# patrickltobing/shallow-wavenet

Hardware: AMD Instinct MI355X
Metric: decoded samples/sec (22.05 kHz Laplacian AR decode, whole job) (higher is better)
Workload: dtype f32

## Files before the change

shallow_wavenet_amd/csrc/swn_decode_bl6w.hip:

```cpp
#include <type_traits>
#include "swn_decode_bl6_common.hpp"
#include "swn_decode_internal.hpp"

namespace {

using namespace swn_bl6;

constexpr int NG = 256;
constexpr int S = 128;
constexpr int O1 = 128;

template <int LPC_, bool EXT_>
struct Tw {
    static constexpr int LPC = LPC_;
    static constexpr bool EXT = EXT_;
    using Ext = Tw<LPC_, true>;
    static constexpr int NO = 2 + LPC_;
    static constexpr int WN = cmax(1, LPC_) + 1;
    static constexpr int ring_len(int l) { return pow2ceil((1 << l) + 1); }
    static constexpr int ring_off(int l) { int o = 0; for (int i = 0; i < l; ++i) o += ring_len(i) * H; return o; }
    static constexpr int PF = L * 2 * H;
    static constexpr int NZC = 64, NZB = 4;
    static constexpr int o_ring = 0;
    static constexpr int o_hcat = o_ring + ring_off(L);
    static constexpr int o_gp = o_hcat + L * H;
    static constexpr int o_bx = o_gp + 2 * PF;
    static constexpr int o_bd = o_bx + L * 2 * H;
    static constexpr int o_old = o_bd + L * 2 * H;
    static constexpr int o_wup = o_old + 2 * L * 2 * H;
    static constexpr int o_skip = o_wup + 256;
    static constexpr int o_p2 = o_skip + S;
    static constexpr int o_tnz = o_p2 + 4 * NO;
    static constexpr int o_cz = o_tnz + r4(NZB * NZC);
    static constexpr int o_w2 = o_cz + 5 * H;
    static constexpr int o_bias = o_w2 + NO * S + r4(NO);
    static constexpr int o_w1 = o_bias + S + O1;
    static constexpr int o_wl = o_w1 + 8 * O1 * 16;
    static constexpr int o_h0w = o_wl + 8 * NG * 4;
    static constexpr int o_end = o_h0w + 3 * H;
    static constexpr size_t lds_bytes = (size_t)o_end * sizeof(float);
    static constexpr int sess_old = ring_off(L);
    static constexpr int sess_win = sess_old + 2 * L * 2 * H;
    static constexpr int sess_floats = sess_win + r4(WN);
};

__device__ __forceinline__ float sum_quads(float v) {
    v += dpp_f<0x124>(v);
    v += dpp_f<0x128>(v);
    float w = v;
    asm("s_nop 1\n\tv_permlane16_swap_b32 %0, %1" : "+v"(v), "+v"(w));
    v += w;
    w = v;
    asm("s_nop 1\n\tv_permlane32_swap_b32 %0, %1" : "+v"(v), "+v"(w));
    return v + w;
}
template <class T, int LAYER>
__device__ __forceinline__ void layer_a(float* lds, const float (&w)[2][16], const int q, const float wj, const int pb, const int po,
                                        const int ta, const float* xr) {
    const int o = ta >> 2, p = ta & 3, pr = p & 1;
    const float e_old = lds[T::o_old + po + LAYER * 2 * H + pr * H + o];
    const float e_gx = fmaf(wj, lds[T::o_gp + pb + LAYER * 2 * H + pr * H + o], lds[T::o_bx + LAYER * 2 * H + pr * H + o]);
    const float e_hp = xr[o];
    float az = 0.f, ac = 0.f;
#pragma unroll
    for (int m = 0; m < 4; ++m) {
        const float4 x = *reinterpret_cast<const float4*>(xr + 16 * p + 4 * m);
        az = fmaf(w[0][4 * m], x.x, az); ac = fmaf(w[1][4 * m], x.x, ac);
        az = fmaf(w[0][4 * m + 1], x.y, az); ac = fmaf(w[1][4 * m + 1], x.y, ac);
        az = fmaf(w[0][4 * m + 2], x.z, az); ac = fmaf(w[1][4 * m + 2], x.z, ac);
        az = fmaf(w[0][4 * m + 3], x.w, az); ac = fmaf(w[1][4 * m + 3], x.w, ac);
    }
    az = sum4(az); ac = sum4(ac);
    __builtin_amdgcn_sched_barrier(0);
    if (p < 2) {
        const float sa = (p == 0 ? az : ac) + e_old;
        const float v = e_gx * sa;
        float res;
        if (fabsf(v) > 9.02f && p == 1) {
            res = copysignf(1.f, v);
        } else {
            const float e = exp_c(p == 0 ? -v : -2.f * fabsf(v));
            const float r = rcp_c(1.f + e);
            res = p == 0 ? r : copysignf((1.f - e) * r, v);
        }
        const float c = dpp_f<0xF5>(res);
        if (p == 0) {
            const float hn = (1.f - res) * c + res * e_hp;
            if (LAYER + 1 < L) {
                constexpr int R2 = T::ring_len(LAYER + 1 < L ? LAYER + 1 : LAYER);
                lds[T::o_ring + T::ring_off(LAYER + 1 < L ? LAYER + 1 : LAYER) + (q & (R2 - 1)) * H + o] = hn;
            }
            lds[T::o_hcat + LAYER * H + o] = hn;
        }
    }
    __builtin_amdgcn_sched_barrier(0);
}

template <class T, int LAYER, int MB = 4>
__device__ __forceinline__ void older_sum(const float* lds, const float (&w)[2][16], const int qn, const int tb, float& az, float& ac) {
    constexpr int dil = 1 << LAYER;
    constexpr int R = T::ring_len(LAYER);
    const int p = tb & 3;
    const float* ring = lds + T::o_ring + T::ring_off(LAYER);
    az = 0.f; ac = 0.f;
#pragma unroll
    for (int m = 0; m < 4; ++m) {
        const float4 x = *reinterpret_cast<const float4*>(ring + ((qn - dil) & (R - 1)) * H + 16 * p + 4 * m);
        float4 w0, w1;
        if (LAYER < L - 1) {
            w0 = make_float4(w[0][4 * m], w[0][4 * m + 1], w[0][4 * m + 2], w[0][4 * m + 3]);
            w1 = make_float4(w[1][4 * m], w[1][4 * m + 1], w[1][4 * m + 2], w[1][4 * m + 3]);
        } else {
            w0 = *reinterpret_cast<const float4*>(lds + T::o_wl + (m * NG + tb) * 4);
            w1 = *reinterpret_cast<const float4*>(lds + T::o_wl + ((4 + m) * NG + tb) * 4);
        }
        az = fmaf(w0.x, x.x, az); ac = fmaf(w1.x, x.x, ac);
        az = fmaf(w0.y, x.y, az); ac = fmaf(w1.y, x.y, ac);
        az = fmaf(w0.z, x.z, az); ac = fmaf(w1.z, x.z, ac);
        az = fmaf(w0.w, x.w, az); ac = fmaf(w1.w, x.w, ac);
        if (MB < 4 && m % MB == MB - 1) __builtin_amdgcn_sched_barrier(0);
    }
    az = sum4(az); ac = sum4(ac);
}
template <class T, int LAYER>
__device__ __forceinline__ void older_store(float* lds, const int qn, const int tb, const float az, const float ac) {
    const int o = tb >> 2, p = tb & 3, pr = p & 1;
    lds[T::o_old + (qn & 1) * (L * 2 * H) + LAYER * 2 * H + pr * H + o] = (p == 0 ? az : ac) + lds[T::o_bd + LAYER * 2 * H + pr * H + o];
}
template <class T, int LAYER, int MB = 4>
__device__ __forceinline__ void older_b(float* lds, const float (&w)[2][16], const int qn, const int tb) {
    float az, ac;
    older_sum<T, LAYER, MB>(lds, w, qn, tb, az, ac);
    if ((tb & 3) < 2) older_store<T, LAYER>(lds, qn, tb, az, ac);
}
template <int... LS> struct Layers {};
template <class T, int NW, int... LS>
__device__ __forceinline__ void older_bn(Layers<LS...>, float* lds, const float (&w)[NW][2][16], const int qn, const int tb) {
    static_assert(((LS < NW) && ...), "register-resident halves only");
    float az[sizeof...(LS)], ac[sizeof...(LS)];
    int k = 0;
    ((older_sum<T, LS>(lds, w[LS], qn, tb, az[k], ac[k]), ++k), ...);
    if ((tb & 3) < 2) {
        k = 0;
        ((older_store<T, LS>(lds, qn, tb, az[k], ac[k]), ++k), ...);
    }
}

template <class T, int LAYER>
__device__ __forceinline__ void older_rows(const float* lds, const int qn, const int tb, float4 (&x)[4]) {
    constexpr int dil = 1 << LAYER;
    constexpr int R = T::ring_len(LAYER);
    const float* row = lds + T::o_ring + T::ring_off(LAYER) + ((qn - dil) & (R - 1)) * H + 16 * (tb & 3);
#pragma unroll
    for (int m = 0; m < 4; ++m) x[m] = *reinterpret_cast<const float4*>(row + 4 * m);
}
__device__ __forceinline__ void older_sum_x(const float (&w)[2][16], const float4 (&x)[4], float& az, float& ac) {
    az = 0.f; ac = 0.f;
#pragma unroll
    for (int m = 0; m < 4; ++m) {
        az = fmaf(w[0][4 * m], x[m].x, az); ac = fmaf(w[1][4 * m], x[m].x, ac);
        az = fmaf(w[0][4 * m + 1], x[m].y, az); ac = fmaf(w[1][4 * m + 1], x[m].y, ac);
        az = fmaf(w[0][4 * m + 2], x[m].z, az); ac = fmaf(w[1][4 * m + 2], x[m].z, ac);
        az = fmaf(w[0][4 * m + 3], x[m].w, az); ac = fmaf(w[1][4 * m + 3], x[m].w, ac);
    }
    az = sum4(az); ac = sum4(ac);
}
template <class T, int... LS>
__device__ __forceinline__ void older_rows_n(Layers<LS...>, const float* lds, const int qn, const int tb, float4 (&x)[sizeof...(LS)][4]) {
    int k = 0;
    ((older_rows<T, LS>(lds, qn, tb, x[k]), ++k), ...);
}
template <class T, int NW, int... LS>
__device__ __forceinline__ void older_bn_x(Layers<LS...>, float* lds, const float (&w)[NW][2][16], const float4 (&x)[sizeof...(LS)][4],
                                           const int qn, const int tb) {
    static_assert(((LS < NW) && ...), "register-resident halves only");
    float az[sizeof...(LS)], ac[sizeof...(LS)];
    int k = 0;
    ((older_sum_x(w[LS], x[k], az[k], ac[k]), ++k), ...);
    if ((tb & 3) < 2) {
        k = 0;
        ((older_store<T, LS>(lds, qn, tb, az[k], ac[k]), ++k), ...);
    }
}

template <int LAYER>
__device__ __forceinline__ void skip_issue_b(__amdgpu_buffer_rsrc_t wsk2, float4 (&wsl)[8], const int tb, const unsigned step0) {
    const int r = tb >> 2, hp = tb & 3;
#pragma unroll
    for (int ps = 0; ps < 2; ++ps)
#pragma unroll
        for (int mm = 0; mm < 4; ++mm)
            wsl[ps * 4 + mm] = buf_ld4(wsk2, (unsigned)((r + 64 * ps) * 4 + hp) * 16u, (unsigned)((LAYER * 4 + mm) * S) * 64u + step0);
}
template <class T, int LAYER>
__device__ __forceinline__ void skip_roll_b(const float* lds, __amdgpu_buffer_rsrc_t wsk2, float4 (&wsl)[8], float (&sacc)[2], const int tb,
                                            const unsigned step0) {
    static_assert(LAYER >= 1 && LAYER < L, "slice LAYER - 1 in flight, slice LAYER to request");
    const int r = tb >> 2, hp = tb & 3;
#pragma unroll
    for (int hf = 0; hf < 2; ++hf) {
#pragma unroll
        for (int mm = 2 * hf; mm < 2 * hf + 2; ++mm) {
            const float4 x = *reinterpret_cast<const float4*>(lds + T::o_hcat + (LAYER - 1) * H + 16 * mm + 4 * hp);
#pragma unroll
            for (int ps = 0; ps < 2; ++ps) {
                const float4 w = wsl[ps * 4 + mm];
                sacc[ps] = fmaf(w.x, x.x, sacc[ps]); sacc[ps] = fmaf(w.y, x.y, sacc[ps]);
                sacc[ps] = fmaf(w.z, x.z, sacc[ps]); sacc[ps] = fmaf(w.w, x.w, sacc[ps]);
            }
        }
        __builtin_amdgcn_sched_barrier(0);
#pragma unroll
        for (int mm = 2 * hf; mm < 2 * hf + 2; ++mm)
#pragma unroll
            for (int ps = 0; ps < 2; ++ps)
                wsl[ps * 4 + mm] = buf_ld4(wsk2, (unsigned)((r + 64 * ps) * 4 + hp) * 16u, (unsigned)((LAYER * 4 + mm) * S) * 64u + step0);
        __builtin_amdgcn_sched_barrier(0);
    }
    asm volatile("" : "+v"(sacc[0]), "+v"(sacc[1]));
}
template <class T>
__device__ __forceinline__ void skip_last_b(float* lds, const float4 (&wsl)[8], const float (&sacc)[2], const int tb) {
    const int r = tb >> 2, hp = tb & 3;
    float part[2][4];
#pragma unroll
    for (int mm = 0; mm < 4; ++mm) {
        const float4 x = *reinterpret_cast<const float4*>(lds + T::o_hcat + (L - 1) * H + 16 * mm + 4 * hp);
#pragma unroll
        for (int ps = 0; ps < 2; ++ps) {
            const float4 w = wsl[ps * 4 + mm];
            part[ps][mm] = fmaf(w.w, x.w, fmaf(w.z, x.z, fmaf(w.y, x.y, w.x * x.x)));
        }
    }
    float s[2];
#pragma unroll
    for (int ps = 0; ps < 2; ++ps) s[ps] = sacc[ps] + ((part[ps][0] + part[ps][1]) + (part[ps][2] + part[ps][3]));
    const float t0 = s[0] + dpp_f<0xB1>(s[0]), t1 = s[1] + dpp_f<0xB1>(s[1]);
    const float v = (hp < 2 ? t0 : t1) + dpp_f<0x4E>(hp < 2 ? t1 : t0);
    if ((hp & 1) == 0) lds[T::o_skip + r + 32 * hp] = fmaxf(v, 0.f);
}

using OlderMerged = Layers<3, 4>;
using OlderOut1 = Layers<0, 1, 2>;

template <class T, bool GA, bool STREAM, bool POOL = false>
__device__ __forceinline__ void decode_body(const Bl6Args& a, float* lds) {
    constexpr bool EXT = T::EXT;
    static_assert(!STREAM || EXT, "streamed chunks run the extended mode");
    constexpr bool grpA = GA;
    const int tid = threadIdx.x, b = POOL ? 0 : blockIdx.x;
    __builtin_assume(GA ? tid < NG : tid >= NG);
    const int tg = tid & (NG - 1);
    const float* __restrict__ P = a.P;
    const int U = a.U;
    const int s0 = STREAM ? a.step0 : 0;
    const bool resume = STREAM && a.resume;
    const int fb0 = STREAM ? s0 / U : 0;

    for (int e = tid; e < T::o_end; e += NT) lds[e] = 0.f;
    __syncthreads();
    for (int e = tid; e < L * 2 * H; e += NT) {
        lds[T::o_bx + e] = P[a.y.bx + e];
        const float bd = P[a.y.bd + e];
        lds[T::o_bd + e] = bd;
        lds[T::o_old + e] = bd;
    }
    for (int e = tid; e < U; e += NT) lds[T::o_wup + e] = P[a.y.wup + e];
    for (int e = tid; e < H; e += NT) lds[T::o_cz + e] = P[a.y.cb + e];
    for (int e = tid; e < S; e += NT) lds[T::o_bias + e] = P[a.y.bsk + e];
    for (int e = tid; e < O1; e += NT) lds[T::o_bias + S + e] = P[a.y.b1 + e];
    for (int e = tid; e < 2 * H; e += NT) { lds[T::o_cz + H + e] = P[a.y.cv + e]; lds[T::o_cz + 3 * H + e] = P[a.y.cc + e]; }
    for (int e = tid; e < T::NO * S; e += NT) lds[T::o_w2 + e] = P[a.y.w2 + (size_t)(e / S) * r4(S) + (e % S)];
    for (int e = tid; e < T::NO; e += NT) lds[T::o_w2 + T::NO * S + e] = P[a.y.b2 + e];
    for (int e = tid; e < 8 * O1 * 16; e += NT) lds[T::o_w1 + e] = P[a.y.w12 + e];
    const __amdgpu_buffer_rsrc_t condr =
        make_rsrc(a.cond + (size_t)b * a.Tf * a.N, (unsigned)((size_t)a.Tf * a.N * sizeof(float)));
    auto load_frame = [&](int fr) {
        float* dst = lds + T::o_gp + (fr & 1) * T::PF;
#pragma unroll
        for (int it = 0; it < (T::PF / 4 + NT - 1) / NT; ++it) {
            const int e4 = it * NT + tid;
            if (e4 < T::PF / 4)
                *reinterpret_cast<float4*>(dst + 4 * e4) =
                    buf_ld4(condr, (unsigned)tid * 16u, (unsigned)(fr * a.N * 4 + it * NT * 16));
        }
    };
    for (int fr = fb0; fr < fb0 + 2 && fr < a.Tf; ++fr) load_frame(fr);
    constexpr int NWR = grpA ? L : L - 1;
    float wreg[NWR][2][16];
    {
        const int o = tg >> 2, p = tg & 3, k = grpA ? 1 : 0;
#pragma unroll
        for (int l = 0; l < L; ++l)
#pragma unroll
            for (int r = 0; r < 2; ++r) {
                const float4* src = reinterpret_cast<const float4*>(P + a.y.wd + (((size_t)l * 2 * H + o + r * H) * 2 + k) * H + 16 * p);
#pragma unroll
                for (int v = 0; v < 4; ++v) {
                    const float4 t = src[v];
                    if (l == L - 1 && !grpA) {
                        *reinterpret_cast<float4*>(lds + T::o_wl + ((r * 4 + v) * NG + tg) * 4) = t;
                    } else {
                        float (&wr)[16] = wreg[l < NWR ? l : 0][r];
                        wr[4 * v] = t.x; wr[4 * v + 1] = t.y; wr[4 * v + 2] = t.z; wr[4 * v + 3] = t.w;
                    }
                }
            }
    }
    __syncthreads();
    const float* sess_b = STREAM ? a.sess + (size_t)b * T::sess_floats : nullptr;
    int tcp = tid;
    asm volatile("" : "+v"(tcp));
    if (resume) {
        for (int e = tcp; e < T::ring_off(L); e += NT) lds[T::o_ring + e] = sess_b[e];
        for (int e = tcp; e < 2 * L * 2 * H; e += NT) lds[T::o_old + e] = sess_b[T::sess_old + e];
        __syncthreads();
    }

    int fb = fb0, tb0 = fb0 * U;
    const int n_pro = RF;
    auto cond_taps = [&](int q, float& wj, int& pb) {
        const int t0 = q - RF;
        const int tlo = t0 < 0 ? 0 : t0;
        if (tlo >= tb0 + U) {
            fb += 1; tb0 += U;
            if (fb + 1 < a.Tf) load_frame(fb + 1);
        }
        int rel = tlo - tb0;
        int fsel = fb;
        if (rel >= U) { rel -= U; fsel = fb + 1; }
        rel = rel < U ? rel : U - 1;
        wj = lds[T::o_wup + rel];
        pb = (fsel & 1) * T::PF;
    };

    auto input_seed = [&](int q) {
        if (tid < H) {
            const int o = tid;
            float acc = c_b;
#pragma unroll
            for (int k = 0; k < 2; ++k) {
                const int r = q - (1 - k);
                if (r >= 0) acc += fmaf(k ? c_v1 : c_v0, 0.f, k ? c_c1 : c_c0);
            }
            lds[T::o_ring + (q & 1) * H + o] = ssign(acc);
        }
    };
    float win[T::WN];
#pragma unroll
    for (int k = 0; k < T::WN; ++k) win[k] = 0.f;
    if (EXT && a.seed) win[T::WN - 1] = reinterpret_cast<const float*>(a.seed)[b];
    if (resume) {
#pragma unroll
        for (int k = 0; k < T::WN; ++k) win[k] = sess_b[T::sess_win + k];
    }
    const int wv = __builtin_amdgcn_readfirstlane(tg >> 6);
    float kcb = 0.f, kv0 = 0.f, kv1 = 0.f, kc0 = 0.f, kc1 = 0.f;
    if (grpA) { const int o = tg & (H - 1); kcb = c_b; kv0 = c_v0; kv1 = c_v1; kc0 = c_c0; kc1 = c_c1; }
    auto h0_row = [&](int qn) -> int {
        return wv == 0 ? T::o_ring + (qn & 1) * H : T::o_h0w + (wv - 1) * H;
    };
    auto input_gen = [&](int row) {
        if constexpr (grpA) {
            float acc = kcb;
            acc += fmaf(kv0, win[T::WN - 2], kc0);
            acc += fmaf(kv1, win[T::WN - 1], kc1);
            lds[row + (tg & (H - 1))] = ssign(acc);
            lds_fence_compiler();
        }
    };
    float e_next = 0.f;
    auto noise_load = [&](int c) {
        const int step = c * T::NZC + tid - 64;
        if (step < a.n_steps) e_next = a.noise[(size_t)b * a.n_steps + step];
    };
    auto noise_chunk = [&](int c) {
        if (grpA && tid >= 64 && tid < 128) {
            const int k = tid - 64, step = c * T::NZC + k;
            if (step < a.n_steps) {
                const float e = EXT ? swn_noise_laplace_at(a.nz, b, step, s0 + step, 0, a.n_steps, 1) : e_next;
                const float sg = (e > 0.f) ? 1.f : ((e < 0.f) ? -1.f : 0.f);
                lds[T::o_tnz + (c & (T::NZB - 1)) * T::NZC + k] = sg * log1pf(-2.f * fabsf(e));
            }
            if (!EXT) noise_load(c + 1);
        }
    };
    if (!EXT && grpA && tid >= 64 && tid < 128) noise_load(0);
    noise_chunk(0);
    noise_chunk(1);

    const __amdgpu_buffer_rsrc_t wsk2 = make_rsrc(P + a.y.wsk2, (unsigned)(L * S * 64 * sizeof(float)));

#ifdef SWN_STAMP
    unsigned long long tw[9] = {0, 0, 0, 0, 0, 0, 0, 0, 0}, tv[6] = {0, 0, 0, 0, 0, 0}, tstep = 0, tlast = 0, tbeg = 0;
#define SWN_BAR(k) { tw[k] += __builtin_amdgcn_s_memtime() - tlast; lds_barrier(); tlast = __builtin_amdgcn_s_memtime(); }
#define SWN_WAIT_STAMP(k) { asm volatile("" :: "v"(wsl[0].x)); tv[k] += __builtin_amdgcn_s_memtime() - tlast; }
#define SWN_PRE(k) { tw[k] += __builtin_amdgcn_s_memtime() - tlast; asm volatile("s_waitcnt lgkmcnt(0)" ::: "memory"); }
#define SWN_BAR_KEEP(k, N) { lds_barrier_keep<N>(); tlast = __builtin_amdgcn_s_memtime(); }
#else
#define SWN_BAR(k) lds_barrier();
#define SWN_WAIT_STAMP(k)
#define SWN_PRE(k)
#define SWN_BAR_KEEP(k, N) lds_barrier_keep<N>();
#endif
#define SWN_PHASE(LAYER, GEN, X0)                                                                                     \
    if constexpr (grpA) layer_a<T, LAYER>(lds, wreg[LAYER], q, wj, pb, po, tg,                                         \
                                          LAYER == 0 ? (X0) : lds + T::o_ring + T::ring_off(LAYER) +                   \
                                                                  (q & (T::ring_len(LAYER) - 1)) * H);                 \
    else {                                                                                                             \
        if (GEN) {    \
                      \
                      \
            if (LAYER == 0) skip_issue_b<0>(wsk2, wsl, tg, step0);                                                     \
            else { SWN_WAIT_STAMP(LAYER > 0 ? LAYER - 1 : 0) skip_roll_b<T, (LAYER > 0 ? LAYER : 1)>(lds, wsk2, wsl, sacc, tg, step0); } \
            __builtin_amdgcn_sched_barrier(0);                                                                         \
        }                                                                                                              \
        if (!(GEN)) older_b<T, LAYER>(lds, wreg[LAYER < NWR ? LAYER : 0], q + 1, tg);                                  \
        else if (LAYER == 0) older_bn<T>(OlderMerged{}, lds, wreg, q + 1, tg);                                         \
        __builtin_amdgcn_sched_barrier(0);                                                                             \
    }                                                                                                                  \
    if (GEN) { SWN_BAR(LAYER) } else lds_barrier();

#pragma unroll 1
    for (int q = resume ? n_pro : 0; q < n_pro; ++q) {
        float wj; int pb;
        float4 wsl[8]; float sacc[2]; const unsigned step0 = 0;
        cond_taps(q, wj, pb);
        const int po = (q & 1) * (L * 2 * H);
        input_seed(q);
        lds_barrier();
        const float* x0 = lds + T::o_ring + (q & 1) * H;
        SWN_PHASE(0, false, x0) SWN_PHASE(1, false, x0) SWN_PHASE(2, false, x0) SWN_PHASE(3, false, x0)
        SWN_PHASE(4, false, x0) SWN_PHASE(5, false, x0)
        (void)wsl; (void)sacc; (void)step0;
    }

    int rel_c = s0 - fb0 * U;
    bool fill_c = false;
    float wj_c = 0.f;
    int pb_c = 0, po_c = 0, x0_c = 0;
    auto taps_ahead = [&](int qn) {
        wj_c = lds[T::o_wup + rel_c];
        pb_c = (fb & 1) * T::PF;
        po_c = (qn & 1) * (L * 2 * H);
        x0_c = h0_row(qn);
        asm volatile("" : "+s"(pb_c), "+s"(po_c), "+s"(x0_c));
    };
    auto frame_advance = [&]() {
        rel_c += 1;
        const bool cross = rel_c >= U;
        if (cross) { rel_c = 0; fb += 1; }
        fill_c = cross && fb + 1 < a.Tf;
    };
    if constexpr (grpA) taps_ahead(RF + s0);
    input_gen(x0_c);
#ifdef SWN_STAMP
    tlast = tbeg = __builtin_amdgcn_s_memtime();
#endif
    auto gen_step = [&](const int i) __attribute__((always_inline)) {
        const int q = RF + s0 + i;
        const float wj = wj_c;
        const int pb = pb_c, po = po_c;
        if constexpr (grpA) {
            if (fill_c) load_frame(fb + 1);
        }
        float4 wsl[8];
        float sacc[2] = {0.f, 0.f};
        if constexpr (!grpA) {
            const float bs0 = lds[T::o_bias + (tg >> 2)], bs1 = lds[T::o_bias + (tg >> 2) + 64];
            if ((tg & 3) == 0) { sacc[0] = bs0; sacc[1] = bs1; }
        }
        unsigned step0 = 0;
        asm volatile("" : "+s"(step0));
        const float* x0 = lds + x0_c;
        SWN_PHASE(0, true, x0) SWN_PHASE(1, true, x0) SWN_PHASE(2, true, x0) SWN_PHASE(3, true, x0)
        SWN_PHASE(4, true, x0) SWN_PHASE(5, true, x0)
        constexpr bool ROLL1 = T::LPC == 0;
        float4 xo[3][4];
        float4 w1e[2][2];
        if constexpr (!grpA) {
            SWN_WAIT_STAMP(5) skip_last_b<T>(lds, wsl, sacc, tg);
            SWN_PRE(6)
            lds_fence_compiler();
            __builtin_amdgcn_sched_barrier(0);
            older_rows_n<T>(OlderOut1{}, lds, q + 1, tg, xo);
            __builtin_amdgcn_sched_barrier(0);
            SWN_BAR_KEEP(6, 12)
        } else {
            older_b<T, L - 1, 2>(lds, wreg[L - 1], q + 1, tg + (int)step0);
            if constexpr (ROLL1) {
                SWN_PRE(6)
                lds_fence_compiler();
                __builtin_amdgcn_sched_barrier(0);
#pragma unroll
                for (int mm = 0; mm < 2; ++mm)
#pragma unroll
                    for (int r = 0; r < 2; ++r)
                        w1e[mm][r] = *reinterpret_cast<const float4*>(lds + T::o_w1 + ((mm * O1 + (tg >> 2) + 64 * r) * 4 + (tg & 3)) * 4);
                __builtin_amdgcn_sched_barrier(0);
                SWN_BAR_KEEP(6, 4)
            } else {
                SWN_BAR(6)
            }
        }
        if constexpr (grpA) {
            const int hr = tg >> 2, hp = tg & 3;
            float a0 = 0.f, a1 = 0.f, b0 = 0.f, b1 = 0.f;
            auto X = [&](int mm) { return *reinterpret_cast<const float4*>(lds + T::o_skip + 16 * mm + 4 * hp); };
            auto W = [&](int mm, int r) { return *reinterpret_cast<const float4*>(lds + T::o_w1 + ((mm * O1 + hr + 64 * r) * 4 + hp) * 4); };
            auto fma8 = [&](int mm, const float4& x0, const float4& w0, const float4& w1) {
                float& acc = (mm & 1) ? a1 : a0;
                float& bcc = (mm & 1) ? b1 : b0;
                acc = fmaf(w0.x, x0.x, acc); acc = fmaf(w0.y, x0.y, acc); acc = fmaf(w0.z, x0.z, acc); acc = fmaf(w0.w, x0.w, acc);
                bcc = fmaf(w1.x, x0.x, bcc); bcc = fmaf(w1.y, x0.y, bcc); bcc = fmaf(w1.z, x0.z, bcc); bcc = fmaf(w1.w, x0.w, bcc);
            };
            float e_b1[2] = {0.f, 0.f}, e_w2[2] = {0.f, 0.f}, e_b2 = 0.f;
            const int e_kc = hp < T::NO ? hp : T::NO - 1;
            if constexpr (ROLL1) {
                static_assert(T::NO <= 4, "one round of out_2 rows");
                float4 xr[3] = {X(0), X(1), X(2)};
                __builtin_amdgcn_sched_barrier(0);
#pragma unroll
                for (int mm = 0; mm < 8; ++mm) {
                    fma8(mm, xr[mm % 3], w1e[mm % 2][0], w1e[mm % 2][1]);
                    __builtin_amdgcn_sched_barrier(0);
                    if (mm + 2 < 8) { w1e[mm % 2][0] = W(mm + 2, 0); w1e[mm % 2][1] = W(mm + 2, 1); }
                    if (mm + 3 < 8) xr[mm % 3] = X(mm + 3);
                    if (mm == 5) {
                        e_b1[0] = lds[T::o_bias + S + hr]; e_b1[1] = lds[T::o_bias + S + hr + 64];
                        e_w2[0] = lds[T::o_w2 + e_kc * S + hr]; e_w2[1] = lds[T::o_w2 + e_kc * S + hr + 64];
                    }
                    if (mm == 6) e_b2 = lds[T::o_w2 + T::NO * S + e_kc];
                    __builtin_amdgcn_sched_barrier(0);
                }
            } else {
#pragma unroll
                for (int mm = 0; mm < 8; ++mm) {
                    fma8(mm, X(mm), W(mm, 0), W(mm, 1));
                    if ((mm & 3) == 3) __builtin_amdgcn_sched_barrier(0);
                }
            }
            const float v = sum4(a0 + a1), u = sum4(b0 + b1);
            if constexpr (ROLL1) {
                const float o1a = fmaxf(v + e_b1[0], 0.f), o1b = fmaxf(u + e_b1[1], 0.f);
                const float pz = sum_quads(fmaf(e_w2[1], o1b, fmaf(e_w2[0], o1a, tg < 4 ? e_b2 : 0.f)));
                if ((tg & 63) < 4 && hp < T::NO) lds[T::o_p2 + 4 * hp + wv] = pz;
            } else {
                const float o1a = fmaxf(v + lds[T::o_bias + S + hr], 0.f), o1b = fmaxf(u + lds[T::o_bias + S + hr + 64], 0.f);
#pragma unroll
                for (int j = 0; j < (T::NO + 3) / 4; ++j) {
                    const int k = hp + 4 * j, kc = k < T::NO ? k : T::NO - 1;
                    const float* w2 = lds + T::o_w2 + kc * S;
                    const float b2 = lds[T::o_w2 + T::NO * S + kc];
                    const float pz = sum_quads(fmaf(w2[hr + 64], o1b, fmaf(w2[hr], o1a, tg < 4 ? b2 : 0.f)));
                    if ((tg & 63) < 4 && k < T::NO) lds[T::o_p2 + 4 * k + wv] = pz;
                }
            }
        } else {
            older_bn_x<T>(OlderOut1{}, lds, wreg, xo, q + 1, tg);
        }
        SWN_BAR(7)
        if constexpr (grpA) {
            const int ln = tg & 63;
            float tz = 0.f;
            if constexpr (!EXT) tz = lds[T::o_tnz + (i & (T::NZB * T::NZC - 1))];
            float fv = 0.f;
            if (a.forced) fv = reinterpret_cast<const float*>(a.forced)[(size_t)b * a.n_steps + i];
            const float4 pz = *reinterpret_cast<const float4*>(lds + T::o_p2 + 4 * (ln < T::NO ? ln : T::NO - 1));
            __builtin_amdgcn_sched_barrier(0);
            frame_advance();
            taps_ahead(q + 1);
            __builtin_amdgcn_sched_barrier(0);
            const float acc = (pz.x + pz.y) + (pz.z + pz.w);
            float o2[T::NO];
#pragma unroll
            for (int k = 0; k < T::NO; ++k) o2[k] = __builtin_bit_cast(float, __builtin_amdgcn_readlane(__builtin_bit_cast(int, acc), k));
            float sv;
            {
#pragma clang fp contract(off)
                const float mu = o2[0];
                const float bsc = sigm(o2[1]);
                float lpv = 0.f;
#pragma unroll
                for (int k = 0; k < T::LPC; ++k) lpv += o2[2 + T::LPC - 1 - k] * win[T::WN - T::LPC + k];
                const float t = bsc * (EXT ? lds[T::o_tnz + ((i >> 6) & (T::NZB - 1)) * T::NZC + (i & (T::NZC - 1))] : tz);
                sv = (T::LPC > 0) ? (lpv + mu) - t : mu - t;
                sv = fminf(fmaxf(sv, -1.f), 1.f);
                float fd = a.forced ? fv : sv;
                asm volatile("" : "+v"(fd));
#pragma unroll
                for (int k = 0; k + 1 < T::WN; ++k) win[k] = win[k + 1];
                win[T::WN - 1] = fd;
            }
            if (i + 1 < a.n_steps) input_gen(x0_c);
            __builtin_amdgcn_sched_barrier(0);
            if (tid == 0) reinterpret_cast<float*>(a.out)[(size_t)b * a.n_steps + (size_t)i] = sv;
            if (HEADS_ON && a.heads && wv == 0 && ln < T::NO) a.heads[((size_t)b * a.n_steps + i) * T::NO + ln] = acc;
        }
#ifdef SWN_STAMP
        if constexpr (grpA) tw[8] += __builtin_amdgcn_s_memtime() - tlast;
#endif
    };
#pragma unroll 1
    for (int i0 = 0; i0 < a.n_steps; i0 += T::NZC) {
        noise_chunk((i0 >> 6) + 2);
        const int iend = i0 + T::NZC < a.n_steps ? i0 + T::NZC : a.n_steps;
#pragma unroll 1
        for (int i = i0; i < iend; ++i) gen_step(i);
    }
#ifdef SWN_STAMP
    { const unsigned long long tn = __builtin_amdgcn_s_memtime(); tw[0] += tn - tlast; tstep = tn - tbeg; }
#endif
    if constexpr (STREAM) {
        __syncthreads();
        float* so = a.sess + (size_t)b * T::sess_floats;
        tcp = tid;
        asm volatile("" : "+v"(tcp));
        for (int e = tcp; e < T::ring_off(L); e += NT) so[e] = lds[T::o_ring + e];
        for (int e = tcp; e < 2 * L * 2 * H; e += NT) so[T::sess_old + e] = lds[T::o_old + e];
        if (tid == 0) {
#pragma unroll
            for (int k = 0; k < T::WN; ++k) so[T::sess_win + k] = win[k];
        }
    }
#undef SWN_PHASE
#undef SWN_BAR
#undef SWN_WAIT_STAMP
#undef SWN_PRE
#undef SWN_BAR_KEEP
#ifdef SWN_STAMP
    if ((tid == 0 || tid == 64 || tid == NG) && b == 0 && a.heads) {
        float* h = a.heads + (tid == 0 ? 0 : tid == 64 ? 30 : 10);
        for (int k = 0; k < 9; ++k) h[k] = (float)((double)tw[k] / (double)a.n_steps);
        if (tid == 0) h[9] = (float)((double)tstep / (double)a.n_steps);
        else if (tid == NG) for (int k = 0; k < 6; ++k) h[10 + k] = (float)((double)tv[k] / (double)a.n_steps);
    }
#endif
}

template <class T, bool STREAM = false>
__global__ __launch_bounds__(NT) void decode_bl6w_kernel(const Bl6Args a) {
    extern __shared__ __attribute__((aligned(16))) float lds[];
    if (threadIdx.x < NG) decode_body<T, true, STREAM>(a, lds);
    else decode_body<T, false, STREAM>(a, lds);
}

template <class T, bool MODELS = false>
__global__ __launch_bounds__(NT) void decode_bl6w_pool_kernel(
    const typename std::conditional<MODELS, Bl6PoolModelsArgs, Bl6PoolArgs>::type p) {
    extern __shared__ __attribute__((aligned(16))) float lds[];
    static_assert(T::EXT, "pools run the extended mode");
    Bl6Args a = p.c;
    if constexpr (MODELS) a.P = swn_pool_model(p.m);
    if (!swn_pool_entry_args(a, p.t, 1, 1, T::NO)) return;
    a.sess += (size_t)swn_pool_slot(p.t) * T::sess_floats;
    if (threadIdx.x < NG) decode_body<T, true, true, true>(a, lds);
    else decode_body<T, false, true, true>(a, lds);
}

bool bl6w_applies(const SwnGeom& g) {
    return g.bl6 && g.U <= 256 && g.U >= 2 && !g.audio_in && g.kind == SWN_KIND_LAPLACE && g.S == 128 && g.O1 == 128 &&
           g.seg == 1 && (g.lpc == 0 || g.lpc == 4);
}

template <class F>
int with_tw(const SwnGeom& g, F&& f) {
    if (!bl6w_applies(g)) return SWN_E_UNSUPPORTED;
    if (g.lpc == 0) return f(Tw<0, false>{});
    return f(Tw<4, false>{});
}

}

int swn_decode_bl6w_run(const SwnDecodeCall& c) {
    const hipStream_t st = c.hip_stream;
    if (c.pool) {
        Bl6PoolModelsArgs p;
        fill_args(p.c, c);
        p.t = *c.pool;
        if (c.models) p.m = *c.models;
        return with_tw(c.g, [&](auto tw) {
            using T = typename decltype(tw)::Ext;
            if (c.models)
                return launch_kernel(decode_bl6w_pool_kernel<T, true>, T::lds_bytes, c.batch, p, st, "swn_decode_pool_chunk_models(bl6w)");
            const Bl6PoolArgs& p1 = p;
            return launch_kernel(decode_bl6w_pool_kernel<T>, T::lds_bytes, c.batch, p1, st, "swn_decode_pool_chunk(bl6w)");
        });
    }
    Bl6Args a;
    fill_args(a, c);
    return with_tw(c.g, [&](auto t) {
        using T = decltype(t);
        using X = typename T::Ext;
        static_assert(T::lds_bytes <= 160 * 1024 && X::lds_bytes <= 160 * 1024, "LDS budget");
        if (c.stream) return launch_kernel(decode_bl6w_kernel<X, true>, X::lds_bytes, a.B, a, st, "swn_decode(bl6w)");
        if (wants_ext(a)) return launch_kernel(decode_bl6w_kernel<X>, X::lds_bytes, a.B, a, st, "swn_decode(bl6w)");
        return launch_kernel(decode_bl6w_kernel<T>, T::lds_bytes, a.B, a, st, "swn_decode(bl6w)");
    });
}

size_t swn_decode_bl6w_session_floats(const SwnGeom& g) {
    int n = 0;
    with_tw(g, [&](auto t) { n = decltype(t)::sess_floats; return SWN_OK; });
    return (size_t)n;
}
```

Measured before the change: 378,000.

## Prefetch last-layer older rows across barrier and trim gate reductions

Replaces the two separate quad reductions in layer_a with a single parity-swapped DPP reduction, and makes the tanh branch-free by clamping |v| before the exp. For LPC==0, the last layer's older-sum input rows and weights are loaded into registers before barrier 5 using a keep-barrier. The remaining half is computed after the barrier, so those LDS reads overlap the barrier wait. The skip roll also loads all hcat rows up front and interleaves weight refills per slice. These changes add register pressure, and the parity trick depends on lane pairing being correct.

Measured after the change: 396,600 (median of 6 runs). +4.9%, better.

```diff
diff --git a/shallow_wavenet_amd/csrc/swn_decode_bl6w.hip b/shallow_wavenet_amd/csrc/swn_decode_bl6w.hip
--- a/shallow_wavenet_amd/csrc/swn_decode_bl6w.hip
+++ b/shallow_wavenet_amd/csrc/swn_decode_bl6w.hip
@@ -54,6 +54,11 @@
     asm("s_nop 1\n\tv_permlane32_swap_b32 %0, %1" : "+v"(v), "+v"(w));
     return v + w;
 }
+__device__ __forceinline__ float quad_sum_by_parity(float own, float other) {
+    float s = own + dpp_f<0xB1>(other);
+    s += dpp_f<0x4E>(s);
+    return s;
+}
 template <class T, int LAYER>
 __device__ __forceinline__ void layer_a(float* lds, const float (&w)[2][16], const int q, const float wj, const int pb, const int po,
                                         const int ta, const float* xr) {
@@ -70,19 +75,14 @@
         az = fmaf(w[0][4 * m + 2], x.z, az); ac = fmaf(w[1][4 * m + 2], x.z, ac);
         az = fmaf(w[0][4 * m + 3], x.w, az); ac = fmaf(w[1][4 * m + 3], x.w, ac);
     }
-    az = sum4(az); ac = sum4(ac);
+    const float sq = quad_sum_by_parity(pr ? ac : az, pr ? az : ac);
     __builtin_amdgcn_sched_barrier(0);
     if (p < 2) {
-        const float sa = (p == 0 ? az : ac) + e_old;
+        const float sa = sq + e_old;
         const float v = e_gx * sa;
-        float res;
-        if (fabsf(v) > 9.02f && p == 1) {
-            res = copysignf(1.f, v);
-        } else {
-            const float e = exp_c(p == 0 ? -v : -2.f * fabsf(v));
-            const float r = rcp_c(1.f + e);
-            res = p == 0 ? r : copysignf((1.f - e) * r, v);
-        }
+        const float e = exp_c(p == 0 ? -v : -2.f * fminf(fabsf(v), 64.f));
+        const float r = rcp_c(1.f + e);
+        const float res = p == 0 ? r : copysignf((1.f - e) * r, v);
         const float c = dpp_f<0xF5>(res);
         if (p == 0) {
             const float hn = (1.f - res) * c + res * e_hp;
@@ -131,6 +131,40 @@
 __device__ __forceinline__ void older_b(float* lds, const float (&w)[2][16], const int qn, const int tb) {
     float az, ac;
     older_sum<T, LAYER, MB>(lds, w, qn, tb, az, ac);
+    if ((tb & 3) < 2) older_store<T, LAYER>(lds, qn, tb, az, ac);
+}
+template <class T>
+__device__ __forceinline__ void older_last_rows(const float* lds, const int qn, const int tb, float4 (&x)[2], float4 (&w)[2][2]) {
+    constexpr int LAYER = L - 1, dil = 1 << LAYER, R = T::ring_len(LAYER);
+    const float* row = lds + T::o_ring + T::ring_off(LAYER) + ((qn - dil) & (R - 1)) * H + 16 * (tb & 3);
+#pragma unroll
+    for (int m = 0; m < 2; ++m) {
+        x[m] = *reinterpret_cast<const float4*>(row + 4 * m);
+        w[m][0] = *reinterpret_cast<const float4*>(lds + T::o_wl + (m * NG + tb) * 4);
+        w[m][1] = *reinterpret_cast<const float4*>(lds + T::o_wl + ((4 + m) * NG + tb) * 4);
+    }
+}
+template <class T>
+__device__ __forceinline__ void older_last_x(float* lds, const float4 (&xe)[2], const float4 (&we)[2][2], const int qn, const int tb) {
+    constexpr int LAYER = L - 1, dil = 1 << LAYER, R = T::ring_len(LAYER);
+    const float* row = lds + T::o_ring + T::ring_off(LAYER) + ((qn - dil) & (R - 1)) * H + 16 * (tb & 3);
+    float az = 0.f, ac = 0.f;
+#pragma unroll
+    for (int m = 0; m < 4; ++m) {
+        float4 x, w0, w1;
+        if (m < 2) { x = xe[m]; w0 = we[m][0]; w1 = we[m][1]; }
+        else {
+            x = *reinterpret_cast<const float4*>(row + 4 * m);
+            w0 = *reinterpret_cast<const float4*>(lds + T::o_wl + (m * NG + tb) * 4);
+            w1 = *reinterpret_cast<const float4*>(lds + T::o_wl + ((4 + m) * NG + tb) * 4);
+        }
+        az = fmaf(w0.x, x.x, az); ac = fmaf(w1.x, x.x, ac);
+        az = fmaf(w0.y, x.y, az); ac = fmaf(w1.y, x.y, ac);
+        az = fmaf(w0.z, x.z, az); ac = fmaf(w1.z, x.z, ac);
+        az = fmaf(w0.w, x.w, az); ac = fmaf(w1.w, x.w, ac);
+        if (m == 1) __builtin_amdgcn_sched_barrier(0);
+    }
+    az = sum4(az); ac = sum4(ac);
     if ((tb & 3) < 2) older_store<T, LAYER>(lds, qn, tb, az, ac);
 }
 template <int... LS> struct Layers {};
@@ -197,24 +231,21 @@
                                             const unsigned step0) {
     static_assert(LAYER >= 1 && LAYER < L, "slice LAYER - 1 in flight, slice LAYER to request");
     const int r = tb >> 2, hp = tb & 3;
-#pragma unroll
-    for (int hf = 0; hf < 2; ++hf) {
-#pragma unroll
-        for (int mm = 2 * hf; mm < 2 * hf + 2; ++mm) {
-            const float4 x = *reinterpret_cast<const float4*>(lds + T::o_hcat + (LAYER - 1) * H + 16 * mm + 4 * hp);
-#pragma unroll
-            for (int ps = 0; ps < 2; ++ps) {
-                const float4 w = wsl[ps * 4 + mm];
-                sacc[ps] = fmaf(w.x, x.x, sacc[ps]); sacc[ps] = fmaf(w.y, x.y, sacc[ps]);
-                sacc[ps] = fmaf(w.z, x.z, sacc[ps]); sacc[ps] = fmaf(w.w, x.w, sacc[ps]);
-            }
+    float4 xs[4];
+#pragma unroll
+    for (int mm = 0; mm < 4; ++mm) xs[mm] = *reinterpret_cast<const float4*>(lds + T::o_hcat + (LAYER - 1) * H + 16 * mm + 4 * hp);
+#pragma unroll
+    for (int mm = 0; mm < 4; ++mm) {
+#pragma unroll
+        for (int ps = 0; ps < 2; ++ps) {
+            const float4 x = xs[mm], w = wsl[ps * 4 + mm];
+            sacc[ps] = fmaf(w.x, x.x, sacc[ps]); sacc[ps] = fmaf(w.y, x.y, sacc[ps]);
+            sacc[ps] = fmaf(w.z, x.z, sacc[ps]); sacc[ps] = fmaf(w.w, x.w, sacc[ps]);
         }
         __builtin_amdgcn_sched_barrier(0);
 #pragma unroll
-        for (int mm = 2 * hf; mm < 2 * hf + 2; ++mm)
-#pragma unroll
-            for (int ps = 0; ps < 2; ++ps)
-                wsl[ps * 4 + mm] = buf_ld4(wsk2, (unsigned)((r + 64 * ps) * 4 + hp) * 16u, (unsigned)((LAYER * 4 + mm) * S) * 64u + step0);
+        for (int ps = 0; ps < 2; ++ps)
+            wsl[ps * 4 + mm] = buf_ld4(wsk2, (unsigned)((r + 64 * ps) * 4 + hp) * 16u, (unsigned)((LAYER * 4 + mm) * S) * 64u + step0);
         __builtin_amdgcn_sched_barrier(0);
     }
     asm volatile("" : "+v"(sacc[0]), "+v"(sacc[1]));
@@ -403,7 +434,7 @@
 #define SWN_PRE(k)
 #define SWN_BAR_KEEP(k, N) lds_barrier_keep<N>();
 #endif
-#define SWN_PHASE(LAYER, GEN, X0)                                                                                     \
+#define SWN_PHASE_WORK(LAYER, GEN, X0)                                                                                \
     if constexpr (grpA) layer_a<T, LAYER>(lds, wreg[LAYER], q, wj, pb, po, tg,                                         \
                                           LAYER == 0 ? (X0) : lds + T::o_ring + T::ring_off(LAYER) +                   \
                                                                   (q & (T::ring_len(LAYER) - 1)) * H);                 \
@@ -418,8 +449,8 @@
         if (!(GEN)) older_b<T, LAYER>(lds, wreg[LAYER < NWR ? LAYER : 0], q + 1, tg);                                  \
         else if (LAYER == 0) older_bn<T>(OlderMerged{}, lds, wreg, q + 1, tg);                                         \
         __builtin_amdgcn_sched_barrier(0);                                                                             \
-    }                                                                                                                  \
-    if (GEN) { SWN_BAR(LAYER) } else lds_barrier();
+    }
+#define SWN_PHASE(LAYER, GEN, X0) SWN_PHASE_WORK(LAYER, GEN, X0) if (GEN) { SWN_BAR(LAYER) } else lds_barrier();
 
 #pragma unroll 1
     for (int q = resume ? n_pro : 0; q < n_pro; ++q) {
@@ -474,7 +505,20 @@
         asm volatile("" : "+s"(step0));
         const float* x0 = lds + x0_c;
         SWN_PHASE(0, true, x0) SWN_PHASE(1, true, x0) SWN_PHASE(2, true, x0) SWN_PHASE(3, true, x0)
-        SWN_PHASE(4, true, x0) SWN_PHASE(5, true, x0)
+        SWN_PHASE(4, true, x0)
+        constexpr bool EARLY5 = T::LPC == 0;
+        float4 xl[2], wl[2][2];
+        SWN_PHASE_WORK(5, true, x0)
+        if constexpr (grpA && EARLY5) {
+            SWN_PRE(5)
+            lds_fence_compiler();
+            __builtin_amdgcn_sched_barrier(0);
+            older_last_rows<T>(lds, q + 1, tg + (int)step0, xl, wl);
+            __builtin_amdgcn_sched_barrier(0);
+            SWN_BAR_KEEP(5, 6)
+        } else {
+            SWN_BAR(5)
+        }
         constexpr bool ROLL1 = T::LPC == 0;
         float4 xo[3][4];
         float4 w1e[2][2];
@@ -487,7 +531,8 @@
             __builtin_amdgcn_sched_barrier(0);
             SWN_BAR_KEEP(6, 12)
         } else {
-            older_b<T, L - 1, 2>(lds, wreg[L - 1], q + 1, tg + (int)step0);
+            if constexpr (EARLY5) older_last_x<T>(lds, xl, wl, q + 1, tg + (int)step0);
+            else older_b<T, L - 1, 2>(lds, wreg[L - 1], q + 1, tg + (int)step0);
             if constexpr (ROLL1) {
                 SWN_PRE(6)
                 lds_fence_compiler();
@@ -624,6 +669,7 @@
         }
     }
 #undef SWN_PHASE
+#undef SWN_PHASE_WORK
 #undef SWN_BAR
 #undef SWN_WAIT_STAMP
 #undef SWN_PRE
```
